# xbpeng/DeepMimic

Hardware: NVIDIA H100
Metric: env-steps/sec (30 Hz policy steps; humanoid3d_spinkick, 4096 envs/GPU) (higher is better)
Workload: dtype f32

## Files before the change

### deepmimic_b200/csrc/kernels/dm_step.cu

```cuda
#include "dm_model.cuh"
#include <type_traits>

namespace dmk {

namespace {

template <int W>
struct Tl {
    static __device__ __forceinline__ float shfl(float v, int src) { return __shfl_sync(0xffffffffu, v, src, W); }
    static __device__ __forceinline__ int shfli(int v, int src) { return __shfl_sync(0xffffffffu, v, src, W); }
    static __device__ __forceinline__ V3 shfl3(V3 v, int src) { return mk3(shfl(v.x, src), shfl(v.y, src), shfl(v.z, src)); }
    static __device__ __forceinline__ S6 shfl6(S6 v, int src) { return mks(shfl3(v.a, src), shfl3(v.l, src)); }
};
__device__ __forceinline__ void ld12(const float* p, float* o) {
    const float4 a = reinterpret_cast<const float4*>(p)[0], b = reinterpret_cast<const float4*>(p)[1], c_ = reinterpret_cast<const float4*>(p)[2];
    o[0] = a.x; o[1] = a.y; o[2] = a.z; o[3] = a.w; o[4] = b.x; o[5] = b.y; o[6] = b.z; o[7] = b.w; o[8] = c_.x; o[9] = c_.y; o[10] = c_.z; o[11] = c_.w;
}
__device__ __forceinline__ void st12(float* p, const float* o) {
    reinterpret_cast<float4*>(p)[0] = make_float4(o[0], o[1], o[2], o[3]); reinterpret_cast<float4*>(p)[1] = make_float4(o[4], o[5], o[6], o[7]);
    reinterpret_cast<float4*>(p)[2] = make_float4(o[8], o[9], o[10], o[11]);
}
__device__ __forceinline__ float rcp_fast(float x) { float r; asm("rcp.approx.ftz.f32 %0, %1;" : "=f"(r) : "f"(x)); return r; }
__device__ __forceinline__ int wmax(int v) {
#pragma unroll
// ... 69 lines not shown
int dm_step_layout(int nl, int n, int chain_len, int maxrows, int W, StepLayout* L) {
    const int maxpts = maxrows / 3;
    int o = 0;
    L->nl = nl; L->n = n; L->chain_len = chain_len; L->maxrows = maxrows; L->maxpts = maxpts;
    L->oU = o; o += nl * 24;
    L->oR = o; o += nl * 12;
    L->oA = o;
    const int world = nl * 24, tri = maxrows * (maxrows + 1) / 2;
    L->oW = o; L->oV = o + nl * 12;
    L->oPp = o + world; L->oQ = L->oPp + maxpts * 4;
    const int pre = world + maxpts * 4 + 4 * 8;
    o += (pre > tri ? pre : tri);
    o = (o + 3) & ~3;
    const int ys = dm_step_y_stride(W), scr = 28 * (nl - 1);
    L->oY = o; o += (chain_len * ys > scr) ? chain_len * ys : scr;
    L->oLam = o; o += maxrows; o += (o & 1); L->oRhs = o; o += maxrows; L->oInv = o; o += maxrows;
    L->oRl = o; o += maxrows;
    L->oPi = o; o += maxpts; L->oPr = o; o += maxpts;
    L->oG = o; o += 21 + 13 + 2;
    L->oZ = o; o += ((n + 3) / 4) * 4;
    L->env_floats = ((o + 15) / 32) * 32 + 16;
    L->hot_floats = kHdrFloats + ((nl * kLkFloats + (nl * nl + nl * chain_len + 3) / 4 + 3) / 4) * 4;
    return L->hot_floats * 4 + 0;
}
int dm_step_smem_bytes(const StepLayout& L, int tiles) { return (L.hot_floats + L.env_floats * tiles) * static_cast<int>(sizeof(float)); }

constexpr int kPgsBlock = 2;
enum PgsSection { kSecLimit = 0, kSecNormal = 1, kSecFriction = 2 };
template <int W, int S, int ST, int B>
__device__ __forceinline__ void pgs_sweeps(const float* sA, float* sLam, const float2* sRI, int lane, int NL, int P, int NLmax, int Pmax, float mu) {
    using T = Tl<W>;
    float w[S];
#pragma unroll
    for (int s = 0; s < S; ++s) w[s] = 0.f;
    int tjs[S];
#pragma unroll
    for (int s = 0; s < S; ++s) { const int rid = lane + s * W; tjs[s] = rid * (rid + 1) / 2; }
    auto tri = [](int i) { return (i * (i + 1)) >> 1; };
    auto a_own = [&](int s, int i, int ti) -> float {
        if (ST > 0) return sA[i * ST + lane + s * W];
        const int rid = lane + s * W;
        return sA[(rid >= i) ? (tjs[s] + i) : (ti + rid)];
    };
    auto a_pair = [&](int i, int j, int ti, int tj_) -> float {
        if (ST > 0) return sA[i * ST + j];
        return sA[(i >= j) ? (ti + j) : (tj_ + i)];
    };
#pragma unroll 1
    for (int p = 0; p < Pmax; ++p) {
        const int i = NL + ((p < P) ? p : 0);
        const float l0 = (p < P) ? sLam[i] : 0.f;
#pragma unroll
        for (int s = 0; s < S; ++s) w[s] = fmaf(a_own(s, i, tri(i)), l0, w[s]);
    }
    bool writer[B];
#pragma unroll
    for (int k = 0; k < B; ++k) writer[k] = lane == k;
    auto block = [&](int pos0, int it, auto sec_tag) {
        constexpr int SEC = decltype(sec_tag)::value;
        int ik[B], tk[B]; bool vk[B];
        float tot = 0.f;
        float wk[B], rhs[B], inv[B], lam[B], lo[B], hi[B], ain[B * (B - 1) / 2 > 0 ? B * (B - 1) / 2 : 1], ao[S][B];
        if (SEC == kSecLimit) {
#pragma unroll
            for (int k = 0; k < B; ++k) { const int pos = pos0 + k; vk[k] = pos < NL; ik[k] = vk[k] ? ((it & 1) ? pos : NL - 1 - pos) : 0; }
        } else {
            const int i0 = ((SEC == kSecNormal) ? NL : NL + P) + pos0, cnt = (SEC == kSecNormal) ? P : 2 * P;
#pragma unroll
            for (int k = 0; k < B; ++k) { ik[k] = i0 + k; vk[k] = pos0 + k < cnt; }
        }
#pragma unroll
        for (int k = 0; k < B; ++k) tk[k] = (ST > 0) ? 0 : tri(ik[k]);
#pragma unroll
        for (int k = 0; k < B; ++k) {
            const float2 ri = sRI[ik[k]];
            rhs[k] = ri.x; inv[k] = ri.y; lam[k] = sLam[ik[k]];
            if (SEC == kSecFriction) {
                if ((B & 1) != 0 || (k & 1) == 0) tot = sLam[NL + ((pos0 + k) >> 1)];
                const bool on = tot > 0.f;
                hi[k] = on ? mu * tot : lam[k]; lo[k] = on ? -hi[k] : lam[k];
            } else { lo[k] = 0.f; hi[k] = (SEC == kSecLimit) ? 100.f : 1e10f; }
        }
        {
            int o = 0;
#pragma unroll
            for (int k = 1; k < B; ++k)
#pragma unroll
                for (int j = 0; j < k; ++j) ain[o++] = a_pair(ik[k], ik[j], tk[k], tk[j]);
        }
#pragma unroll
        for (int s = 0; s < S; ++s)
#pragma unroll
            for (int k = 0; k < B; ++k) ao[s][k] = a_own(s, ik[k], tk[k]);
#pragma unroll
        for (int k = 0; k < B; ++k) {
            float sel = w[0];
#pragma unroll
            for (int s = 1; s < S; ++s) if (ik[k] >= s * W) sel = w[s];
            wk[k] = T::shfl(sel, (S == 1) ? ik[k] : (ik[k] & (W - 1)));
        }
#pragma unroll
        for (int k = 0; k < B; ++k) {
            float c = fmaxf(fmaf(-inv[k], wk[k], rhs[k]), lo[k] - lam[k]);
            if (SEC != kSecNormal) c = fminf(c, hi[k] - lam[k]);
            c = vk[k] ? c : 0.f;
#pragma unroll
            for (int j = k + 1; j < B; ++j) wk[j] = fmaf(ain[j * (j - 1) / 2 + k], c, wk[j]);
            if (vk[k] && writer[k]) sLam[ik[k]] = (SEC == kSecNormal) ? fmaxf(lam[k] + c, 0.f) : fminf(fmaxf(lam[k] + c, lo[k]), hi[k]);
#pragma unroll
            for (int s = 0; s < S; ++s) w[s] = fmaf(ao[s][k], c, w[s]);
        }
        __syncwarp();
    };
#pragma unroll 1
    for (int it = 0; it < 10; ++it) {
#pragma unroll 1
        for (int p0 = 0; p0 < NLmax; p0 += B) block(p0, it, std::integral_constant<int, kSecLimit>{});
#pragma unroll 1
        for (int p0 = 0; p0 < Pmax; p0 += B) block(p0, it, std::integral_constant<int, kSecNormal>{});
#pragma unroll 1
        for (int p0 = 0; p0 < 2 * Pmax; p0 += B) block(p0, it, std::integral_constant<int, kSecFriction>{});
    }
}

template <int W>
__device__ __noinline__ void solve_rows(int NL, int P, float* mani, int alive, unsigned int* prf) {
    using T = Tl<W>;
    float* const sm_ = step_smem();
    const int* LYS = reinterpret_cast<const int*>(sm_ + kHLayout);
    const float* LK = sm_ + kHdrFloats;
    const int lane = threadIdx.x % W;
    const float h = sm_[kHh], mu = sm_[kHMu];
#ifdef DM_PROFILE
    unsigned int pt = static_cast<unsigned int>(clock64());
#define SPROF(sec) do { if ((threadIdx.x & 31) == 0) { unsigned int t_ = static_cast<unsigned int>(clock64()); prf[sec] += t_ - pt; pt = t_; } } while (0)
#else
#define SPROF(sec) do { } while (0)
#endif
    const StepLayout& LY = *reinterpret_cast<const StepLayout*>(LYS);
    const int nl = LY.nl, CL = LY.chain_len, MR = LY.maxrows;
    constexpr int YS = dm_step_y_stride(W);
    float* const E = sm_ + LY.hot_floats + (threadIdx.x / W) * LY.env_floats;
    const unsigned char* CD = reinterpret_cast<const unsigned char*>(LK + nl * kLkFloats);
    const unsigned char* CH = CD + nl * nl;
    float* sU = E + LY.oU; float* sS = E + LY.oR; float* sW = E + LY.oW; float* sV = E + LY.oV; float* sA = E + LY.oA; float* sY = E + LY.oY;
    float* sLam = E + LY.oLam; float2* sRI = reinterpret_cast<float2*>(E + LY.oRhs); int* sRl = reinterpret_cast<int*>(E + LY.oRl);
    float* sPp = E + LY.oPp; float* sPi = E + LY.oPi; int* sPr = reinterpret_cast<int*>(E + LY.oPr);
    float* sQ = E + LY.oQ; float* sG = E + LY.oG; float* sZ = E + LY.oZ;
    auto lk_i = [&](int j) { return reinterpret_cast<const int*>(LK + j * kLkFloats)[kLInt]; };
    auto lk_i2 = [&](int j) { return reinterpret_cast<const int*>(LK + j * kLkFloats)[kLInt2]; };
    auto shift_f = [](S6 f, V3 c) { return mks(f.a + cross(c, f.l), f.l); };
    const int NR = NL + 3 * P;
    const int NRmax = (W == 32) ? NR : wmax(NR);
    const int nslots = (NRmax + W - 1) / W;
    constexpr int kSlots = 2;
#pragma unroll
    for (int s = 0; s < kSlots; ++s) {
        const int rid = lane + s * W;
        if (s < nslots) {
            const bool rv_ = rid < NR;
            int b = 0, kind = 0 , p = 0;
            float lsign = 1.f, lpen = 0.f;
            if (rv_) {
                if (rid < NL) { b = __float_as_int(sQ[rid]); lsign = sQ[8 + rid]; lpen = sQ[16 + rid]; }
                else if (rid < NL + P) { kind = 1; p = rid - NL; b = sPr[p] >> 2; }
                else { const int f = rid - NL - P; p = f >> 1; kind = 2 + (f & 1); b = sPr[p] >> 2; }
                sRl[rid] = b;
            }
            S6 f = mks(mk3(0, 0, 0), mk3(0, 0, 0));
            float rvel = 0.f, pdist = 0.f;
            if (rv_ && kind != 0) {
                const float* w = sW + b * 12;
                pdist = sPp[p * 4 + 3];
                const V3 rel = mk3(sPp[p * 4] - w[9], sPp[p * 4 + 1] - w[10], sPp[p * 4 + 2] - w[11]);
                const V3 fl_ = (kind == 1) ? mk3(0.f, 1.f, 0.f) : ((kind == 2) ? mk3(-1.f, 0.f, 0.f) : mk3(0.f, 0.f, 1.f));
                f = mks(cross(rel, fl_), fl_);
                const float* v = sV + b * 12;
                rvel = dot(fl_, mk3(v[3], v[4], v[5]) + cross(mk3(v[0], v[1], v[2]), rel));
            }
            float acc = 0.f;
            int cur = b;
            bool first = true;
#pragma unroll 1
            while (true) {
                const int info = lk_i(cur);
                const int par = static_cast<int>(static_cast<signed char>(info & 0xff)), nd = (info >> 16) & 0xff, dp0 = (info >> 24) & 0xff;
                const float4* u4 = reinterpret_cast<const float4*>(sU + cur * 24);
                const float4* q4 = reinterpret_cast<const float4*>(sS + cur * 12);
                const float4 ua = u4[0], ub = u4[1], uc = u4[2], ud = u4[3], ue = u4[4], uf = u4[5];
                const float4 qa = q4[0], qb = q4[1], qc = q4[2];
                if (nd == 3) {
                    {
                        const float t = qb.z * f.a.x + qb.w * f.a.y + qc.x * f.a.z;
                        const float y = t * uf.w;
                        if (rv_) sY[(dp0 + 2) * YS + rid] = y;
                        acc += y * y;
                        const float ti = t * uf.x;
                        f.a.x -= ti * ud.x; f.a.y -= ti * ud.y; f.a.z -= ti * ud.z; f.l.x -= ti * ud.w; f.l.y -= ti * ue.x; f.l.z -= ti * ue.y;
                    }
                    {
                        const float t = qa.w * f.a.x + qb.x * f.a.y + qb.y * f.a.z;
                        const float y = t * uf.z;
                        if (rv_) sY[(dp0 + 1) * YS + rid] = y;
                        acc += y * y;
                        const float ti = t * ue.w;
                        f.a.x -= ti * ub.z; f.a.y -= ti * ub.w; f.a.z -= ti * uc.x; f.l.x -= ti * uc.y; f.l.y -= ti * uc.z; f.l.z -= ti * uc.w;
                    }
                }
                if (nd >= 1) {
                    float t = qa.x * f.a.x + qa.y * f.a.y + qa.z * f.a.z;
                    if (first && kind == 0) { t = lsign; rvel = lsign * sQ[24 + rid]; }
                    const float y = t * uf.y;
                    if (rv_) sY[dp0 * YS + rid] = y;
                    acc += y * y;
                    const float ti = t * ue.z;
                    f.a.x -= ti * ua.x; f.a.y -= ti * ua.y; f.a.z -= ti * ua.z; f.l.x -= ti * ua.w; f.l.y -= ti * ub.x; f.l.z -= ti * ub.y;
                }
                first = false;
                f = shift_f(f, mk3(qc.y, qc.z, qc.w));
                if (par < 0) break;
                cur = par;
            }
            {
                float x[6] = {f.a.x, f.a.y, f.a.z, f.l.x, f.l.y, f.l.z};
                int o = 0;
#pragma unroll
                for (int i = 0; i < 6; ++i) {
#pragma unroll
                    for (int k = 0; k < i; ++k) x[i] -= sG[o++] * x[k];
                    x[i] *= sG[15 + i];
                    if (rv_) sY[i * YS + rid] = x[i];
                    acc += x[i] * x[i];
                }
            }
            if (rv_) {
                const float inv = acc > 1.1920929e-7f ? 1.0f / acc : 0.f;
                float rhs, lam0 = 0.f;
                if (kind == 1) {
                    float perr = 0.f, verr = -rvel;
                    if (pdist > 0.f) verr -= pdist / h; else perr = -pdist * 0.2f / h;
                    rhs = perr * inv + verr * inv;
                    lam0 = sPi[p] * 0.85f;
                } else if (kind != 0) rhs = -rvel * inv;
                else {
                    float perr = 0.f, verr = -rvel;
                    const bool combine = lpen > -0.04f;
                    if (lpen > 0.f) verr = -lpen / h; else perr = -lpen * 0.2f / h;
                    rhs = combine ? (perr * inv + verr * inv) : (verr * inv);
                }
                sRI[rid] = make_float2(rhs, inv); sLam[rid] = lam0;
            }
        }
    }
    __syncwarp();
    SPROF(7);
    const int Pmax = (W == 32) ? P : wmax(P);
    const int NLmax = (W == 32) ? NL : wmax(NL);
    {
        constexpr int kSq2 = (W == 16) ? 22 : 36;
        const int region = max(nl * 24, MR * (MR + 1) / 2);
        const int mode = (nslots == 1) ? 0 : ((NRmax <= kSq2 && kSq2 * kSq2 + W <= region) ? 1 : 2);
        const int st = (mode == 0) ? W : kSq2;
        auto put = [&](int i, int j, float v) {
            if (mode != 2) { sA[i * st + j] = v; sA[j * st + i] = v; }
            else { const int hi_ = max(i, j), lo_ = min(i, j); sA[hi_ * (hi_ + 1) / 2 + lo_] = v; }
        };
#pragma unroll 1
        for (int j = 0; j < NLmax; ++j) {
            const bool jv = j < NL;
            const int bj = jv ? sRl[j] : 0;
#pragma unroll 1
            for (int i0 = 0; i0 < NRmax; i0 += W) {
                const int i = i0 + lane;
                const bool pv = jv && i < NR && i >= j;
                const int cd = pv ? CD[sRl[i] * nl + bj] : 0;
                const float* yi = sY + (pv ? i : 0); const float* yj = sY + (jv ? j : 0);
                float acc = 0.f;
#pragma unroll 1
                for (int k = 0; k < CL; k += 4, yi += 4 * YS, yj += 4 * YS) {
                    const float a0 = yi[0], a1 = yi[YS], a2 = yi[2 * YS], a3 = yi[3 * YS];
                    const float b0 = yj[0], b1 = yj[YS], b2 = yj[2 * YS], b3 = yj[3 * YS];
                    if (k < cd) acc += a0 * b0;
                    if (k + 1 < cd) acc += a1 * b1;
                    if (k + 2 < cd) acc += a2 * b2;
                    if (k + 3 < cd) acc += a3 * b3;
                }
                if (pv) put(i, j, acc);
            }
        }
        const int npp = P * (P + 1) / 2, nppmax = Pmax * (Pmax + 1) / 2;
#pragma unroll 1
        for (int q0 = 0; q0 < nppmax; q0 += W) {
            const int q = q0 + lane;
            const bool pv = q < npp;
            int pp = static_cast<int>((sqrtf(8.0f * static_cast<float>(q) + 1.0f) - 1.0f) * 0.5f);
            if (pp * (pp + 1) / 2 > q) --pp;
            if ((pp + 1) * (pp + 2) / 2 <= q) ++pp;
            const int pr = q - pp * (pp + 1) / 2;
            const int in_p = pv ? NL + pp : 0, it_p = pv ? NL + P + 2 * pp : 0, in_r = pv ? NL + pr : 0, it_r = pv ? NL + P + 2 * pr : 0;
            const int cd = pv ? CD[sRl[in_p] * nl + sRl[in_r]] : 0;
            const float* ypn = sY + in_p; const float* ypt = sY + it_p; const float* yrn = sY + in_r; const float* yrt = sY + it_r;
            float acc[3][3];
#pragma unroll
            for (int x = 0; x < 3; ++x)
#pragma unroll
                for (int y = 0; y < 3; ++y) acc[x][y] = 0.f;
#pragma unroll 1
            for (int k = 0; k < CL; k += 4, ypn += 4 * YS, ypt += 4 * YS, yrn += 4 * YS, yrt += 4 * YS) {
                float av[3][4], bv[3][4];
#pragma unroll
                for (int d = 0; d < 4; ++d) {
                    av[0][d] = ypn[d * YS]; av[1][d] = ypt[d * YS]; av[2][d] = ypt[d * YS + 1];
                    bv[0][d] = yrn[d * YS]; bv[1][d] = yrt[d * YS]; bv[2][d] = yrt[d * YS + 1];
                }
#pragma unroll
                for (int d = 0; d < 4; ++d)
                    if (k + d < cd) {
#pragma unroll
                        for (int x = 0; x < 3; ++x)
#pragma unroll
                            for (int y = 0; y < 3; ++y) acc[x][y] += av[x][d] * bv[y][d];
                    }
            }
            if (pv) {
                if (mode != 2) {
                    float* rp[3] = {sA + in_p * st, sA + it_p * st, sA + it_p * st + st};
                    float* rr[3] = {sA + in_r * st, sA + it_r * st, sA + it_r * st + st};
                    const int cp[3] = {in_p, it_p, it_p + 1}, cr[3] = {in_r, it_r, it_r + 1};
#pragma unroll
                    for (int x = 0; x < 3; ++x)
#pragma unroll
                        for (int y = 0; y < 3; ++y) { rp[x][cr[y]] = acc[x][y]; rr[y][cp[x]] = acc[x][y]; }
                } else {
#pragma unroll
                    for (int x = 0; x < 3; ++x)
#pragma unroll
                        for (int y = 0; y < 3; ++y) put(x == 0 ? in_p : it_p + x - 1, y == 0 ? in_r : it_r + y - 1, acc[x][y]);
                }
            }
        }
        __syncwarp();
        SPROF(8);
        if (mode == 0) pgs_sweeps<W, 1, W, kPgsBlock>(sA, sLam, sRI, lane, NL, P, NLmax, Pmax, mu);
        else if (mode == 1) pgs_sweeps<W, kSlots, kSq2, kPgsBlock>(sA, sLam, sRI, lane, NL, P, NLmax, Pmax, mu);
        else pgs_sweeps<W, kSlots, 0, kPgsBlock>(sA, sLam, sRI, lane, NL, P, NLmax, Pmax, mu);
    }
    SPROF(9);
#pragma unroll 1
    for (int p = lane; p < P; p += W) {
        if (alive) {
            const int ref = sPr[p];
            float* mpt = mani + (ref >> 2) * kManifoldFloats + (ref & 3) * 12;
            mpt[7] = sLam[NL + p]; mpt[8] = sLam[NL + P + 2 * p]; mpt[9] = sLam[NL + P + 2 * p + 1];
        }
    }
    {
        const int info = (lane < nl) ? lk_i(lane) : 0;
        const int nd = (info >> 16) & 0xff, dp0 = (info >> 24) & 0xff;
        const int d0 = (lane < nl) ? (lk_i2(lane) & 0xff) : 0;
        float z0 = 0.f, z1 = 0.f, z2 = 0.f, zb = 0.f;
        const int kb = (lane < 6) ? lane : 0;
        const bool mine = lane < nl && nd > 0;
        const int need = dp0 + nd - 1;
        const unsigned char* cdl = CD + lane;
#pragma unroll 2
        for (int i = 0; i < NRmax; ++i) {
            const int b = sRl[i];
            const float l = (i < NR) ? sLam[i] : 0.f;
            const float yb = sY[kb * YS + i], y0 = sY[dp0 * YS + i], y1 = sY[(dp0 + 1) * YS + i], y2 = sY[(dp0 + 2) * YS + i];
            const bool in = mine && cdl[b * nl] > need;
            zb = fmaf(yb, l, zb);
            if (in) { z0 = fmaf(y0, l, z0); if (nd == 3) { z1 = fmaf(y1, l, z1); z2 = fmaf(y2, l, z2); } }
        }
        if (lane < 6) sZ[lane] = zb;
        if (lane < nl && nd >= 1) sZ[d0] = z0;
        if (lane < nl && nd == 3) { sZ[d0 + 1] = z1; sZ[d0 + 2] = z2; }
    }
    __syncwarp();
}


struct Ctx {
    float* E;
    const int* LYS;
    const float* LK;
    int lane, li;
    int plane, level, ndof, jtype, maxlevel;
    bool act;
};
__device__ __forceinline__ const StepLayout& lay_of(const Ctx& c) { return *reinterpret_cast<const StepLayout*>(c.LYS); }
template <int W>
__device__ __forceinline__ Ctx make_ctx() {
    Ctx c;
    float* sm = step_smem();
    c.LYS = reinterpret_cast<const int*>(sm + kHLayout); c.LK = sm + kHdrFloats;
    const StepLayout& LY = *reinterpret_cast<const StepLayout*>(c.LYS);
    const int tile = threadIdx.x / W;
    c.lane = threadIdx.x % W;
    c.act = c.lane < LY.nl;
    c.li = c.act ? c.lane : LY.nl - 1;
    c.E = sm + LY.hot_floats + tile * LY.env_floats;
    const int* q = reinterpret_cast<const int*>(c.LK + c.li * kLkFloats);
    const int info = q[kLInt], tree = q[kLTree];
    const int par = static_cast<int>(static_cast<signed char>(info & 0xff));
    c.plane = par >= 0 ? par : 0; c.jtype = (info >> 8) & 0xff; c.ndof = c.act ? ((info >> 16) & 0xff) : 0;
    c.level = c.act ? (tree & 0xff) : 1000; c.maxlevel = (tree >> 8) & 0xff;
    return c;
}
__device__ __forceinline__ S6 shift_m(S6 m, V3 c) { return mks(m.a, m.l + cross(m.a, c)); }
__device__ __forceinline__ S6 shift_f(S6 f, V3 c) { return mks(f.a + cross(c, f.l), f.l); }
__device__ __forceinline__ float cl100(float v) { return fminf(fmaxf(v, -100.f), 100.f); }
template <int W>
__device__ __forceinline__ V3 tile_com(const float* w, const float* v, float mass, float inv_total) {
    float cx = mass * (w[9] + v[6]), cy = mass * (w[10] + v[7]), cz = mass * (w[11] + v[8]);
#pragma unroll
    for (int o = W / 2; o > 0; o >>= 1) {
        cx += __shfl_xor_sync(0xffffffffu, cx, o, W); cy += __shfl_xor_sync(0xffffffffu, cy, o, W); cz += __shfl_xor_sync(0xffffffffu, cz, o, W);
    }
    return mk3(cx * inv_total, cy * inv_total, cz * inv_total);
}

template <int W>
__device__ __noinline__ void kin_pass(float4 jp, float4 jv) {
    const Ctx c = make_ctx<W>();
    using T = Tl<W>;
    const StepLayout& LY = lay_of(c);
    float* sS = c.E + LY.oR; float* sW = c.E + LY.oW; float* sV = c.E + LY.oV; const float* sB = c.E + LY.oG + 21;
    const float* LKo = c.LK + c.li * kLkFloats;
    const float4 ax4 = ld4(LKo + kLAx), zr4 = ld4(LKo + kLZr), c4 = ld4(LKo + kLC);
    const V3 axis = mk3(ax4.x, ax4.y, ax4.z);
    const Q4 zrot = mkq(zr4.x, zr4.y, zr4.z, zr4.w);
    const V3 cvec = mk3(c4.x, c4.y, c4.z);
    Q4 cached;
    if (c.jtype == kJSpherical) cached = qmul(mkq(jp.x, jp.y, jp.z, -jp.w), zrot);
    else if (c.jtype == kJRevolute) {
        float s, co;
        __sincosf(-0.5f * jp.x, &s, &co);
        cached = qmul(mkq(axis.x * s, axis.y * s, axis.z * s, co), zrot);
    } else cached = zrot;
    const M3 R = qmat(cached);
    V3 jw = mk3(0, 0, 0);
    if (c.jtype == kJSpherical) jw = mk3(jv.x, jv.y, jv.z); else if (c.jtype == kJRevolute) jw = jv.x * axis;
    M3 Rwl; V3 Pw, cw; S6 vel;
    if (c.lane == 0) {
        const M3 Rwb = qmat(mkq(sB[3], sB[4], sB[5], sB[6]));
        const V3 bo = mk3(sB[7], sB[8], sB[9]);
        Rwl = mul(R, Rwb); cw = mulT(Rwb, cvec); Pw = mk3(sB[0], sB[1], sB[2]) + cw;
        vel = mks(bo + mulT(Rwl, jw), mk3(sB[10], sB[11], sB[12]) + cross(bo, cw));
    }
#pragma unroll 1
    for (int lv = 1; lv <= c.maxlevel; ++lv) {
        M3 pR; V3 pp; S6 pv;
#pragma unroll
        for (int k = 0; k < 9; ++k) pR.m[k] = T::shfl(Rwl.m[k], c.plane);
        pp = T::shfl3(Pw, c.plane);
        pv = T::shfl6(vel, c.plane);
        if (c.level == lv) {
            Rwl = mul(R, pR); cw = mulT(pR, cvec); Pw = pp + cw;
            vel = mks(pv.a + mulT(Rwl, jw), pv.l + cross(pv.a, cw));
        }
    }
    if (c.act) {
        const float4 d4 = ld4(LKo + kLD);
        const V3 dw = mulT(Rwl, mk3(d4.x, d4.y, d4.z));
        V3 S0 = mk3(Rwl.m[0], Rwl.m[1], Rwl.m[2]);
        if (c.jtype != kJSpherical) S0 = mulT(Rwl, axis);
        const float wr[12] = {Rwl.m[0], Rwl.m[1], Rwl.m[2], Rwl.m[3], Rwl.m[4], Rwl.m[5], Rwl.m[6], Rwl.m[7], Rwl.m[8], Pw.x, Pw.y, Pw.z};
        const float qr[12] = {S0.x, S0.y, S0.z, Rwl.m[3], Rwl.m[4], Rwl.m[5], Rwl.m[6], Rwl.m[7], Rwl.m[8], cw.x, cw.y, cw.z};
        const float vr[12] = {vel.a.x, vel.a.y, vel.a.z, vel.l.x, vel.l.y, vel.l.z, dw.x, dw.y, dw.z, 0.f, 0.f, 0.f};
        st12(sW + c.lane * 12, wr); st12(sS + c.lane * 12, qr); st12(sV + c.lane * 12, vr);
    }
    __syncwarp();
}

template <int W>
__device__ __noinline__ int collide(float* mani, int alive, int mcnt) {
    const Ctx c = make_ctx<W>();
    const float scale = step_smem()[kHScale];
    using T = Tl<W>;
    const StepLayout& LY = lay_of(c);
    const float* sW = c.E + LY.oW; const float* sV = c.E + LY.oV;
    float* sPp = c.E + LY.oPp; float* sPi = c.E + LY.oPi; int* sPr = reinterpret_cast<int*>(c.E + LY.oPr);
    const float* LKo = c.LK + c.li * kLkFloats;
    const int shape = reinterpret_cast<const int*>(LKo)[kLFlg] & 0xff;
    int cnt = 0;
    float mp[48];
    M3 Rwl;
    float wrec[12], vrec[12];
    ld12(sW + c.li * 12, wrec); ld12(sV + c.li * 12, vrec);
#pragma unroll
    for (int k = 0; k < 9; ++k) Rwl.m[k] = wrec[k];
    const float thr = LKo[kLThr];
    const float4 he4 = ld4(LKo + kLHe);
    const V3 he = mk3(he4.x, he4.y, he4.z);
    const V3 pos = mk3(wrec[9] + vrec[6], wrec[10] + vrec[7], wrec[11] + vrec[8]);
    V3 dl = mul(Rwl, mk3(0.f, -1.f, 0.f));
    V3 vtx;
    if (shape == kSBox) vtx = mk3(dl.x >= 0 ? he.x : -he.x, dl.y >= 0 ? he.y : -he.y, dl.z >= 0 ? he.z : -he.z);
    else {
        V3 sup = mk3(0, 0, 0);
        if (shape == kSCapsule) sup = mk3(0.f, (dl.y >= 0.f) ? he.y : -he.y, 0.f);
        float inv = rsqrtf(dot(dl, dl));
        vtx = sup + (he.x * inv) * dl;
    }
    const V3 vw = pos + mulT(Rwl, vtx);
    const float dist = vw.y;
    const bool need = c.act && alive && (mcnt > 0 || dist < thr);
    {
        const float4* mg = reinterpret_cast<const float4*>(mani + c.li * kManifoldFloats);
#pragma unroll
        for (int k = 0; k < 12; ++k) { float4 v = need ? mg[k] : make_float4(0.f, 0.f, 0.f, 0.f); mp[4 * k] = v.x; mp[4 * k + 1] = v.y; mp[4 * k + 2] = v.z; mp[4 * k + 3] = v.w; }
    }
#pragma unroll
    for (int k = 0; k < 4; ++k) if (mp[k * 12] != 0.f && cnt == k) cnt = k + 1;
    if (c.act && dist < thr) {
        float best = thr * thr; int nearest = -1;
#pragma unroll
        for (int k = 0; k < 4; ++k) if (k < cnt) {
// ... 562 lines not shown
                    if (kind == kTaskStrike) {
                        const double scene_time = tm[kTTimer];
                        tk[kKTimer] += dt;
                        strike_update(M.taskx, tk, tkx, rx, rz, scene_time, B);
                        if (tk[kKTimer] >= tk[kKTimerMax]) task_timer_reset(M.task, tk, rng);
                        tf = strike_terminate(M.task, M.taskx, tk, tkx, rx, rz, scene_time);
                    } else {
                        task_update(task_base_kind(kind), M.task, tk, rng, dt, rx, rz);
                        tf = task_dist_fail(kind, M.task, tk, rx, rz) ? 1 : 0;
                        if (kind == kTaskHeadingGetup) {
                            tkx[kXHeadY] = B.head_y;
                            if (getup_update(M.taskx, tkx, dt, M.test_mode != 0, fallen != 0)) fe = 0;
                        }
                    }
                }
                task_fail = T::shfli(tf, 0);
                fallen_eff = T::shfli(fe, 0);
            }
            if (alive) {
                int term = (M.enable_fall_end && fallen_eff) ? 1 : 0;
                if (!term && (cbits & 4)) term = 1;
                if (TASK && !term && task_fail) term = task_fail;
                f_updates++;
                const bool end = (cbits & 2) || term;
                if (end || stage == total_stages) {
                    if (lane == 0) {
                        reinterpret_cast<float4*>(sim)[0] = make_float4(sB[0], sB[1], sB[2], 0.f);
                        reinterpret_cast<float4*>(sim)[1] = make_float4(sB[3], sB[4], sB[5], sB[6]);
                        reinterpret_cast<float4*>(sim)[2] = make_float4(sB[7], sB[8], sB[9], 0.f);
                        reinterpret_cast<float4*>(sim)[3] = make_float4(sB[10], sB[11], sB[12], 0.f);
                        fl[kFNeedAction] = need_action; fl[kFDone] = end ? 1 : 0; fl[kFTerminate] = term; fl[kFValid] = (eseg == 0) ? 1 : 0; fl[kFFallen] = fallen_eff;
                        fl[kFRowOverflow] = f_over; fl[kFUpdates] = f_updates;
                    }
                    if (act) {
                        reinterpret_cast<float4*>(sim + 16)[lane] = jp;
                        reinterpret_cast<float4*>(sim + 16 + 4 * nl)[lane] = jv;
                    }
                }
                if (end) alive = false;
            }
        }
        PROF(1);
        if (stage == total_stages) break;
        if (__syncthreads_and(!alive)) break;
        PROF(2);
        if (__ballot_sync(0xffffffffu, alive) == 0u) continue;
        const int ph = stage % stages_per_upd;
        if (ph == 0) {
            int cb = 0;
            if constexpr (TASK) {
                if (__ballot_sync(0xffffffffu, alive && need_action) != 0u) {
                    const V3 com = tile_com<W>(E + LY.oW + li * 12, sV + li * 12, act ? LKo[kLM] : 0.f, 1.0f / (M.total_mass * scale));
                    if (lane == 0 && alive && need_action) { tk[kKPrevCom] = com.x; tk[kKPrevCom + 1] = com.y; tk[kKPrevCom + 2] = com.z; }
                }
            }
            if (lane == 0 && alive) {
                const double timer = tm[kTTimer] + dt;
                double kin_time = tm[kTKin];
                double dur_ = M.motion_dur;
                if constexpr (TASK) dur_ = st.ctab->info[st.clip[env]].dur;
                const double dur = dur_;
                double p0 = kin_time / dur; p0 -= floor(p0);
                kin_time += dt;
                double p1 = kin_time / dur; p1 -= floor(p1);
                if constexpr (TASK) {
                    const ClipInfo& ci = st.ctab->info[st.clip[env]];
                    if (ci.loop && p1 < p0 && M.sync_root_pos) {
                        const double simq[4] = {static_cast<double>(sB[3]), static_cast<double>(sB[4]), static_cast<double>(sB[5]), static_cast<double>(sB[6])};
                        kin_wrap_sync(frame_times + ci.frame_off, frames + static_cast<size_t>(ci.frame_off) * M.pose_dim, M.pose_dim, ci.num_frames, ci.cycle_delta, dur, kin_time,
                                      tm + kTOrigin, tm + kTOriginRot, static_cast<double>(sB[0]) / M.scale, static_cast<double>(sB[2]) / M.scale, simq, true, false);
                    }
                } else if (M.loop_motion && p1 < p0 && (M.sync_root_pos || M.sync_root_rot)) {
                    const double simq[4] = {static_cast<double>(sB[3]), static_cast<double>(sB[4]), static_cast<double>(sB[5]), static_cast<double>(sB[6])};
                    kin_wrap_sync(frame_times, frames, M.pose_dim, M.num_frames, M.cycle_delta, dur, kin_time, tm + kTOrigin, tm + kTOriginRot,
                                  static_cast<double>(sB[0]) / M.scale, static_cast<double>(sB[2]) / M.scale, simq, M.sync_root_pos != 0, M.sync_root_rot != 0);
                }
                const double ctrl_time = tm[kTCtrl] + dt;
                if (need_action) tm[kTPrevAct] = ctrl_time;
                tm[kTTimer] = timer; tm[kTKin] = kin_time; tm[kTCtrl] = ctrl_time;
                {
                    const double cur = ctrl_time + tm[kTInitOff], pad = 0.001 * dt, T_ = M.query_dt;
                    int c0 = static_cast<int>(floor((cur + pad) / T_)), c1 = static_cast<int>(floor((cur + pad - dt) / T_));
                    cb = (c0 != c1) ? 1 : 0;
                }
                if (timer >= tm[kTTimerMax]) cb |= 2;
                if (M.end_at_clip_end && kin_time >= dur) cb |= 4;
            }
            cbits = T::shfli(cb, 0);
            need_action = 0;
            PROF(3);
            const float4 tg = reinterpret_cast<const float4*>(sim + 16 + 8 * nl)[li];
            float e0 = 0, e1 = 0, e2 = 0;
            if (jtype == kJSpherical) {
                Q4 q = mkq(jp.x, jp.y, jp.z, jp.w);
                Q4 dq = qmul(q, mkq(jv.x, jv.y, jv.z, 0.f));
                Q4 qi = qnormalize(mkq(q.x + 0.5f * fdt * dq.x, q.y + 0.5f * fdt * dq.y, q.z + 0.5f * fdt * dq.z, q.w + 0.5f * fdt * dq.w));
                V3 e = quat_rotvec3(qmul(qconj(qi), mkq(tg.x, tg.y, tg.z, tg.w)));
                e0 = e.x; e1 = e.y; e2 = e.z;
            } else if (jtype == kJRevolute) {
                e0 = tg.x - (normalize_angle3(jp.x) + fdt * jv.x);
            }
            const float kp = LKo[kLKp], kd = LKo[kLKd];
            const float pe0 = kp * e0, pe1 = kp * e1, pe2 = kp * e2;
            const float3 qdd = aba_solve<W>(pe0 - kd * jv.x, pe1 - kd * jv.y, pe2 - kd * jv.z, fdt * kd, 0, jv.x, jv.y, jv.z);
            float t0 = 0, t1 = 0, t2 = 0;
            if (ndof >= 1) t0 = pe0 + kd * (-jv.x - fdt * qdd.x);
            if (ndof == 3) { t1 = pe1 + kd * (-jv.y - fdt * qdd.y); t2 = pe2 + kd * (-jv.z - fdt * qdd.z); }
            const float mag = sqrtf(t0 * t0 + t1 * t1 + t2 * t2), tlim = LKo[kLTl];
            if (mag > tlim) { float s = tlim / mag; t0 *= s; t1 *= s; t2 *= s; }
            tau0 = t0; tau1 = t1; tau2 = t2;
            PROF(4);
            continue;
        }
        int P;
        {
            const int r = collide<W>(mani, alive ? 1 : 0, mcnt);
            P = r & 0xff; in_contact_tol = ((r >> 8) & 1) != 0; if ((r >> 9) & 1) f_over = 1; mcnt = (r >> 10) & 7;
        }
        PROF(3);
        {
            const float3 qdd = aba_solve<W>(tau0, tau1, tau2, 0.f, 1, jv.x, jv.y, jv.z);
            bool hit = false;
            if (ndof >= 1) { const float v = jv.x + h * qdd.x; jv.x = cl100(v); hit |= fabsf(v) > 100.f; }
            if (ndof == 3) { const float v1 = jv.y + h * qdd.y, v2 = jv.z + h * qdd.z; jv.y = cl100(v1); jv.z = cl100(v2); hit |= fabsf(v1) > 100.f || fabsf(v2) > 100.f; }
            if (lane == 0) for (int k = 0; k < 6; ++k) hit |= fabsf(sB[7 + k]) >= 100.f;
            const unsigned hb = __ballot_sync(0xffffffffu, hit);
            if (hb != 0u) {
                const unsigned hseg = (W == 32) ? hb : ((hb >> (threadIdx.x & 16)) & 0xffffu);
                vel_pass<W>(jv.x, jv.y, jv.z, hseg != 0u);
            }
        }
        PROF(4);
        int lim_dir = 0; float lim_pen = 0.f;
        if (act && has_limit && alive) {
            float p0 = jp.x - LKo[kLLo], p1 = LKo[kLHi] - jp.x;
            if (!(p0 > 0.f)) { lim_dir = 1; lim_pen = p0; }
            else if (!(p1 > 0.f)) { lim_dir = -1; lim_pen = p1; }
        }
        const unsigned lbal = __ballot_sync(0xffffffffu, lim_dir != 0);
        const unsigned lseg = (W == 32) ? lbal : ((lbal >> (threadIdx.x & 16)) & 0xffffu);
        int NL = __popc(lseg);
        const unsigned anyrow = __ballot_sync(0xffffffffu, NL + P > 0);
        if (anyrow != 0) {
            {
                const int lidx = __popc(lseg & ((1u << lane) - 1u));
                if (NL > 8) { NL = 8; f_over = 1; }
                if (lim_dir != 0 && lidx < 8) { sQ[lidx] = __int_as_float(lane); sQ[8 + lidx] = (lim_dir == -1) ? -1.f : 1.f; sQ[16 + lidx] = lim_pen; sQ[24 + lidx] = jv.x; }
            }
            if (NL + 3 * P > LY.maxrows) { P = (LY.maxrows - NL) / 3; f_over = 1; }
            const int NR = NL + 3 * P;
            __syncwarp();
            PROF(5);
#ifdef DM_PROFILE
            { const int nrm = wmax(NR); if ((threadIdx.x & 31) == 0) { PRF[13] += nrm; PRF[14] += 1; if (nrm > W) PRF[15] += 1; } }
#endif
            solve_rows<W>(NL, P, mani, alive ? 1 : 0, PRFP);
            PROF(10);
            const float3 dq = dv_pass<W>();
            if (NR > 0) {
                if (ndof >= 1) jv.x = cl100(jv.x + dq.x);
                if (ndof == 3) { jv.y = cl100(jv.y + dq.y); jv.z = cl100(jv.z + dq.z); }
            }
            PROF(11);
        }
        if (lane == 0) {
            sB[0] += h * sB[10]; sB[1] += h * sB[11]; sB[2] += h * sB[12];
            const Q4 q = quat_integrate3(mk3(sB[7], sB[8], sB[9]), mkq(sB[3], sB[4], sB[5], sB[6]), true, h);
            sB[3] = q.x; sB[4] = q.y; sB[5] = q.z; sB[6] = q.w;
        }
        if (jtype == kJRevolute) jp.x += h * jv.x;
        else if (jtype == kJSpherical) { Q4 q = quat_integrate3(mk3(jv.x, jv.y, jv.z), mkq(jp.x, jp.y, jp.z, jp.w), false, h); jp = make_float4(q.x, q.y, q.z, q.w); }
        __syncwarp();
        need_kin = true;
        if (ph == sim_substeps) pending_flags = true;
        PROF(12);
    }
#ifdef DM_PROFILE
    __syncwarp();
    if ((threadIdx.x & 31) == 0 && st.prof) { unsigned int* o = st.prof + (blockIdx.x * (blockDim.x / 32) + threadIdx.x / 32) * kProfCounters; for (int k = 0; k < kProfCounters; ++k) o[k] = PRF[k]; }
#endif
}

template __global__ void dm_step_kernel<16, false>(const DevModel*, DevState, const double*, const float*, double, int, int, StepLayout);
template __global__ void dm_step_kernel<32, false>(const DevModel*, DevState, const double*, const float*, double, int, int, StepLayout);
template __global__ void dm_step_kernel<16, true>(const DevModel*, DevState, const double*, const float*, double, int, int, StepLayout);
template __global__ void dm_step_kernel<32, true>(const DevModel*, DevState, const double*, const float*, double, int, int, StepLayout);

}
```

Before: 2.342 million.

## Solve each half-warp env serially with full warp when rows exceed half-warp

In the W=16 half-warp-per-env path, when one env has more constraint rows than 16 but both fit in 32, the warp now processes the two envs one after another using all 32 lanes. This avoids the two-slot row layout and packed/square-matrix PGS modes with half-warp granularity, using a single-slot 32-wide PGS instead. Row building and A assembly are refactored into lambdas parameterized on the env base pointer. It also raises the unroll of the impulse accumulation loop for W=16; the trade-off is serializing two envs, which can cost time when both envs have many rows.

Result: faster. 2.409 million, median of 6 (+2.8%).

```diff
diff --git a/deepmimic_b200/csrc/kernels/dm_step.cu b/deepmimic_b200/csrc/kernels/dm_step.cu
--- a/deepmimic_b200/csrc/kernels/dm_step.cu
+++ b/deepmimic_b200/csrc/kernels/dm_step.cu
@@ -245,129 +245,124 @@
     auto shift_f = [](S6 f, V3 c) { return mks(f.a + cross(c, f.l), f.l); };
     const int NR = NL + 3 * P;
     const int NRmax = (W == 32) ? NR : wmax(NR);
-    const int nslots = (NRmax + W - 1) / W;
-    constexpr int kSlots = 2;
-#pragma unroll
-    for (int s = 0; s < kSlots; ++s) {
-        const int rid = lane + s * W;
-        if (s < nslots) {
-            const bool rv_ = rid < NR;
-            int b = 0, kind = 0 , p = 0;
-            float lsign = 1.f, lpen = 0.f;
-            if (rv_) {
-                if (rid < NL) { b = __float_as_int(sQ[rid]); lsign = sQ[8 + rid]; lpen = sQ[16 + rid]; }
-                else if (rid < NL + P) { kind = 1; p = rid - NL; b = sPr[p] >> 2; }
-                else { const int f = rid - NL - P; p = f >> 1; kind = 2 + (f & 1); b = sPr[p] >> 2; }
-                sRl[rid] = b;
-            }
-            S6 f = mks(mk3(0, 0, 0), mk3(0, 0, 0));
-            float rvel = 0.f, pdist = 0.f;
-            if (rv_ && kind != 0) {
-                const float* w = sW + b * 12;
-                pdist = sPp[p * 4 + 3];
-                const V3 rel = mk3(sPp[p * 4] - w[9], sPp[p * 4 + 1] - w[10], sPp[p * 4 + 2] - w[11]);
-                const V3 fl_ = (kind == 1) ? mk3(0.f, 1.f, 0.f) : ((kind == 2) ? mk3(-1.f, 0.f, 0.f) : mk3(0.f, 0.f, 1.f));
-                f = mks(cross(rel, fl_), fl_);
-                const float* v = sV + b * 12;
-                rvel = dot(fl_, mk3(v[3], v[4], v[5]) + cross(mk3(v[0], v[1], v[2]), rel));
-            }
-            float acc = 0.f;
-            int cur = b;
-            bool first = true;
-#pragma unroll 1
-            while (true) {
-                const int info = lk_i(cur);
-                const int par = static_cast<int>(static_cast<signed char>(info & 0xff)), nd = (info >> 16) & 0xff, dp0 = (info >> 24) & 0xff;
-                const float4* u4 = reinterpret_cast<const float4*>(sU + cur * 24);
-                const float4* q4 = reinterpret_cast<const float4*>(sS + cur * 12);
-                const float4 ua = u4[0], ub = u4[1], uc = u4[2], ud = u4[3], ue = u4[4], uf = u4[5];
-                const float4 qa = q4[0], qb = q4[1], qc = q4[2];
-                if (nd == 3) {
-                    {
-                        const float t = qb.z * f.a.x + qb.w * f.a.y + qc.x * f.a.z;
-                        const float y = t * uf.w;
-                        if (rv_) sY[(dp0 + 2) * YS + rid] = y;
-                        acc += y * y;
-                        const float ti = t * uf.x;
-                        f.a.x -= ti * ud.x; f.a.y -= ti * ud.y; f.a.z -= ti * ud.z; f.l.x -= ti * ud.w; f.l.y -= ti * ue.x; f.l.z -= ti * ue.y;
-                    }
-                    {
-                        const float t = qa.w * f.a.x + qb.x * f.a.y + qb.y * f.a.z;
-                        const float y = t * uf.z;
-                        if (rv_) sY[(dp0 + 1) * YS + rid] = y;
-                        acc += y * y;
-                        const float ti = t * ue.w;
-                        f.a.x -= ti * ub.z; f.a.y -= ti * ub.w; f.a.z -= ti * uc.x; f.l.x -= ti * uc.y; f.l.y -= ti * uc.z; f.l.z -= ti * uc.w;
-                    }
+    auto in_blk = [&](float* Eb, int off, float* own) -> float* { if constexpr (W == 16) return Eb + off; else return own; };
+    auto build_row = [&](float* Eb, int rid, bool rv_, int NL, int P) {
+        const float* sUe = in_blk(Eb, LY.oU, sU); const float* sSe = in_blk(Eb, LY.oR, sS); const float* sWe = in_blk(Eb, LY.oW, sW);
+        const float* sVe = in_blk(Eb, LY.oV, sV); const float* sPpe = in_blk(Eb, LY.oPp, sPp); const float* sPie = in_blk(Eb, LY.oPi, sPi);
+        const int* sPre = reinterpret_cast<const int*>(in_blk(Eb, LY.oPr, reinterpret_cast<float*>(sPr))); const float* sQe = in_blk(Eb, LY.oQ, sQ);
+        const float* sGe = in_blk(Eb, LY.oG, sG); float* sYe = in_blk(Eb, LY.oY, sY); float* sLame = in_blk(Eb, LY.oLam, sLam);
+        float2* sRIe = reinterpret_cast<float2*>(in_blk(Eb, LY.oRhs, reinterpret_cast<float*>(sRI))); int* sRle = reinterpret_cast<int*>(in_blk(Eb, LY.oRl, reinterpret_cast<float*>(sRl)));
+        int b = 0, kind = 0 , p = 0;
+        float lsign = 1.f, lpen = 0.f;
+        if (rv_) {
+            if (rid < NL) { b = __float_as_int(sQe[rid]); lsign = sQe[8 + rid]; lpen = sQe[16 + rid]; }
+            else if (rid < NL + P) { kind = 1; p = rid - NL; b = sPre[p] >> 2; }
+            else { const int f = rid - NL - P; p = f >> 1; kind = 2 + (f & 1); b = sPre[p] >> 2; }
+            sRle[rid] = b;
+        }
+        S6 f = mks(mk3(0, 0, 0), mk3(0, 0, 0));
+        float rvel = 0.f, pdist = 0.f;
+        if (rv_ && kind != 0) {
+            const float* w = sWe + b * 12;
+            pdist = sPpe[p * 4 + 3];
+            const V3 rel = mk3(sPpe[p * 4] - w[9], sPpe[p * 4 + 1] - w[10], sPpe[p * 4 + 2] - w[11]);
+            const V3 fl_ = (kind == 1) ? mk3(0.f, 1.f, 0.f) : ((kind == 2) ? mk3(-1.f, 0.f, 0.f) : mk3(0.f, 0.f, 1.f));
+            f = mks(cross(rel, fl_), fl_);
+            const float* v = sVe + b * 12;
+            rvel = dot(fl_, mk3(v[3], v[4], v[5]) + cross(mk3(v[0], v[1], v[2]), rel));
+        }
+        float acc = 0.f;
+        int cur = b;
+        bool first = true;
+#pragma unroll 1
+        while (true) {
+            const int info = lk_i(cur);
+            const int par = static_cast<int>(static_cast<signed char>(info & 0xff)), nd = (info >> 16) & 0xff, dp0 = (info >> 24) & 0xff;
+            const float4* u4 = reinterpret_cast<const float4*>(sUe + cur * 24);
+            const float4* q4 = reinterpret_cast<const float4*>(sSe + cur * 12);
+            const float4 ua = u4[0], ub = u4[1], uc = u4[2], ud = u4[3], ue = u4[4], uf = u4[5];
+            const float4 qa = q4[0], qb = q4[1], qc = q4[2];
+            if (nd == 3) {
+                {
+                    const float t = qb.z * f.a.x + qb.w * f.a.y + qc.x * f.a.z;
+                    const float y = t * uf.w;
+                    if (rv_) sYe[(dp0 + 2) * YS + rid] = y;
+                    acc += y * y;
+                    const float ti = t * uf.x;
+                    f.a.x -= ti * ud.x; f.a.y -= ti * ud.y; f.a.z -= ti * ud.z; f.l.x -= ti * ud.w; f.l.y -= ti * ue.x; f.l.z -= ti * ue.y;
                 }
-                if (nd >= 1) {
-                    float t = qa.x * f.a.x + qa.y * f.a.y + qa.z * f.a.z;
-                    if (first && kind == 0) { t = lsign; rvel = lsign * sQ[24 + rid]; }
-                    const float y = t * uf.y;
-                    if (rv_) sY[dp0 * YS + rid] = y;
+                {
+                    const float t = qa.w * f.a.x + qb.x * f.a.y + qb.y * f.a.z;
+                    const float y = t * uf.z;
+                    if (rv_) sYe[(dp0 + 1) * YS + rid] = y;
                     acc += y * y;
-                    const float ti = t * ue.z;
-                    f.a.x -= ti * ua.x; f.a.y -= ti * ua.y; f.a.z -= ti * ua.z; f.l.x -= ti * ua.w; f.l.y -= ti * ub.x; f.l.z -= ti * ub.y;
+                    const float ti = t * ue.w;
+                    f.a.x -= ti * ub.z; f.a.y -= ti * ub.w; f.a.z -= ti * uc.x; f.l.x -= ti * uc.y; f.l.y -= ti * uc.z; f.l.z -= ti * uc.w;
                 }
-                first = false;
-                f = shift_f(f, mk3(qc.y, qc.z, qc.w));
-                if (par < 0) break;
-                cur = par;
-            }
-            {
-                float x[6] = {f.a.x, f.a.y, f.a.z, f.l.x, f.l.y, f.l.z};
-                int o = 0;
-#pragma unroll
-                for (int i = 0; i < 6; ++i) {
-#pragma unroll
-                    for (int k = 0; k < i; ++k) x[i] -= sG[o++] * x[k];
-                    x[i] *= sG[15 + i];
-                    if (rv_) sY[i * YS + rid] = x[i];
-                    acc += x[i] * x[i];
-                }
-            }
-            if (rv_) {
-                const float inv = acc > 1.1920929e-7f ? 1.0f / acc : 0.f;
-                float rhs, lam0 = 0.f;
-                if (kind == 1) {
-                    float perr = 0.f, verr = -rvel;
-                    if (pdist > 0.f) verr -= pdist / h; else perr = -pdist * 0.2f / h;
-                    rhs = perr * inv + verr * inv;
-                    lam0 = sPi[p] * 0.85f;
-                } else if (kind != 0) rhs = -rvel * inv;
-                else {
-                    float perr = 0.f, verr = -rvel;
-                    const bool combine = lpen > -0.04f;
-                    if (lpen > 0.f) verr = -lpen / h; else perr = -lpen * 0.2f / h;
-                    rhs = combine ? (perr * inv + verr * inv) : (verr * inv);
-                }
-                sRI[rid] = make_float2(rhs, inv); sLam[rid] = lam0;
-            }
-        }
-    }
-    __syncwarp();
-    SPROF(7);
-    const int Pmax = (W == 32) ? P : wmax(P);
-    const int NLmax = (W == 32) ? NL : wmax(NL);
-    {
-        constexpr int kSq2 = (W == 16) ? 22 : 36;
-        const int region = max(nl * 24, MR * (MR + 1) / 2);
-        const int mode = (nslots == 1) ? 0 : ((NRmax <= kSq2 && kSq2 * kSq2 + W <= region) ? 1 : 2);
+            }
+            if (nd >= 1) {
+                float t = qa.x * f.a.x + qa.y * f.a.y + qa.z * f.a.z;
+                if (first && kind == 0) { t = lsign; rvel = lsign * sQe[24 + rid]; }
+                const float y = t * uf.y;
+                if (rv_) sYe[dp0 * YS + rid] = y;
+                acc += y * y;
+                const float ti = t * ue.z;
+                f.a.x -= ti * ua.x; f.a.y -= ti * ua.y; f.a.z -= ti * ua.z; f.l.x -= ti * ua.w; f.l.y -= ti * ub.x; f.l.z -= ti * ub.y;
+            }
+            first = false;
+            f = shift_f(f, mk3(qc.y, qc.z, qc.w));
+            if (par < 0) break;
+            cur = par;
+        }
+        {
+            float x[6] = {f.a.x, f.a.y, f.a.z, f.l.x, f.l.y, f.l.z};
+            int o = 0;
+#pragma unroll
+            for (int i = 0; i < 6; ++i) {
+#pragma unroll
+                for (int k = 0; k < i; ++k) x[i] -= sGe[o++] * x[k];
+                x[i] *= sGe[15 + i];
+                if (rv_) sYe[i * YS + rid] = x[i];
+                acc += x[i] * x[i];
+            }
+        }
+        if (rv_) {
+            const float inv = acc > 1.1920929e-7f ? 1.0f / acc : 0.f;
+            float rhs, lam0 = 0.f;
+            if (kind == 1) {
+                float perr = 0.f, verr = -rvel;
+                if (pdist > 0.f) verr -= pdist / h; else perr = -pdist * 0.2f / h;
+                rhs = perr * inv + verr * inv;
+                lam0 = sPie[p] * 0.85f;
+            } else if (kind != 0) rhs = -rvel * inv;
+            else {
+                float perr = 0.f, verr = -rvel;
+                const bool combine = lpen > -0.04f;
+                if (lpen > 0.f) verr = -lpen / h; else perr = -lpen * 0.2f / h;
+                rhs = combine ? (perr * inv + verr * inv) : (verr * inv);
+            }
+            sRIe[rid] = make_float2(rhs, inv); sLame[rid] = lam0;
+        }
+    };
+    constexpr int kSq2 = (W == 16) ? 22 : 36;
+    const int region = max(nl * 24, MR * (MR + 1) / 2);
+    auto build_A = [&](float* Eb, int ln, int nlanes, int NL, int P, int NR, int NLmax, int Pmax, int NRmax, int mode) {
+        float* sAe = in_blk(Eb, LY.oA, sA); const float* sYe = in_blk(Eb, LY.oY, sY); const int* sRle = reinterpret_cast<const int*>(in_blk(Eb, LY.oRl, reinterpret_cast<float*>(sRl)));
         const int st = (mode == 0) ? W : kSq2;
         auto put = [&](int i, int j, float v) {
-            if (mode != 2) { sA[i * st + j] = v; sA[j * st + i] = v; }
-            else { const int hi_ = max(i, j), lo_ = min(i, j); sA[hi_ * (hi_ + 1) / 2 + lo_] = v; }
+            if (mode != 2) { sAe[i * st + j] = v; sAe[j * st + i] = v; }
+            else { const int hi_ = max(i, j), lo_ = min(i, j); sAe[hi_ * (hi_ + 1) / 2 + lo_] = v; }
         };
 #pragma unroll 1
         for (int j = 0; j < NLmax; ++j) {
             const bool jv = j < NL;
-            const int bj = jv ? sRl[j] : 0;
-#pragma unroll 1
-            for (int i0 = 0; i0 < NRmax; i0 += W) {
-                const int i = i0 + lane;
+            const int bj = jv ? sRle[j] : 0;
+#pragma unroll 1
+            for (int i0 = 0; i0 < NRmax; i0 += nlanes) {
+                const int i = i0 + ln;
                 const bool pv = jv && i < NR && i >= j;
-                const int cd = pv ? CD[sRl[i] * nl + bj] : 0;
-                const float* yi = sY + (pv ? i : 0); const float* yj = sY + (jv ? j : 0);
+                const int cd = pv ? CD[sRle[i] * nl + bj] : 0;
+                const float* yi = sYe + (pv ? i : 0); const float* yj = sYe + (jv ? j : 0);
                 float acc = 0.f;
 #pragma unroll 1
                 for (int k = 0; k < CL; k += 4, yi += 4 * YS, yj += 4 * YS) {
@@ -383,16 +378,16 @@
         }
         const int npp = P * (P + 1) / 2, nppmax = Pmax * (Pmax + 1) / 2;
 #pragma unroll 1
-        for (int q0 = 0; q0 < nppmax; q0 += W) {
-            const int q = q0 + lane;
+        for (int q0 = 0; q0 < nppmax; q0 += nlanes) {
+            const int q = q0 + ln;
             const bool pv = q < npp;
             int pp = static_cast<int>((sqrtf(8.0f * static_cast<float>(q) + 1.0f) - 1.0f) * 0.5f);
             if (pp * (pp + 1) / 2 > q) --pp;
             if ((pp + 1) * (pp + 2) / 2 <= q) ++pp;
             const int pr = q - pp * (pp + 1) / 2;
             const int in_p = pv ? NL + pp : 0, it_p = pv ? NL + P + 2 * pp : 0, in_r = pv ? NL + pr : 0, it_r = pv ? NL + P + 2 * pr : 0;
-            const int cd = pv ? CD[sRl[in_p] * nl + sRl[in_r]] : 0;
-            const float* ypn = sY + in_p; const float* ypt = sY + it_p; const float* yrn = sY + in_r; const float* yrt = sY + it_r;
+            const int cd = pv ? CD[sRle[in_p] * nl + sRle[in_r]] : 0;
+            const float* ypn = sYe + in_p; const float* ypt = sYe + it_p; const float* yrn = sYe + in_r; const float* yrt = sYe + it_r;
             float acc[3][3];
 #pragma unroll
             for (int x = 0; x < 3; ++x)
@@ -417,8 +412,8 @@
             }
             if (pv) {
                 if (mode != 2) {
-                    float* rp[3] = {sA + in_p * st, sA + it_p * st, sA + it_p * st + st};
-                    float* rr[3] = {sA + in_r * st, sA + it_r * st, sA + it_r * st + st};
+                    float* rp[3] = {sAe + in_p * st, sAe + it_p * st, sAe + it_p * st + st};
+                    float* rr[3] = {sAe + in_r * st, sAe + it_r * st, sAe + it_r * st + st};
                     const int cp[3] = {in_p, it_p, it_p + 1}, cr[3] = {in_r, it_r, it_r + 1};
 #pragma unroll
                     for (int x = 0; x < 3; ++x)
@@ -433,12 +428,53 @@
             }
         }
         __syncwarp();
+    };
+    bool serial = false;
+    if constexpr (W == 16) serial = NRmax > W && -wmax(-NR) <= W;
+    if (serial) {
+        if constexpr (W == 16) {
+            const int lw = threadIdx.x & 31;
+#pragma unroll 1
+            for (int e = 0; e < 2; ++e) {
+                const int NLe = __shfl_sync(0xffffffffu, NL, 16 * e), Pe = __shfl_sync(0xffffffffu, P, 16 * e), NRe = NLe + 3 * Pe;
+                if (NRe == 0) continue;
+                float* const Ee = sm_ + LY.hot_floats + ((threadIdx.x >> 5) * 2 + e) * LY.env_floats;
+                build_row(Ee, lw, lw < NRe, NLe, Pe);
+                __syncwarp();
+                SPROF(7);
+                const int mode = (NRe <= kSq2 && kSq2 * kSq2 + 32 <= region) ? 1 : 2;
+                build_A(Ee, lw, 32, NLe, Pe, NRe, NLe, Pe, NRe, mode);
+                SPROF(8);
+                const float2* RIe = reinterpret_cast<const float2*>(Ee + LY.oRhs);
+                if (mode == 1) pgs_sweeps<32, 1, kSq2, kPgsBlock>(Ee + LY.oA, Ee + LY.oLam, RIe, lw, NLe, Pe, NLe, Pe, mu);
+                else pgs_sweeps<32, 1, 0, kPgsBlock>(Ee + LY.oA, Ee + LY.oLam, RIe, lw, NLe, Pe, NLe, Pe, mu);
+                SPROF(9);
+            }
+        }
+    } else {
+        const int nslots = (NRmax + W - 1) / W;
+        constexpr int kSlots = 2;
+#pragma unroll
+        for (int s = 0; s < kSlots; ++s) {
+            const int rid = lane + s * W;
+            if (s < nslots) build_row(E, rid, rid < NR, NL, P);
+        }
+        __syncwarp();
+        SPROF(7);
+        const int Pmax = (W == 32) ? P : wmax(P);
+        const int NLmax = (W == 32) ? NL : wmax(NL);
+        const int mode = (nslots == 1) ? 0 : ((NRmax <= kSq2 && kSq2 * kSq2 + W <= region) ? 1 : 2);
+        build_A(E, lane, W, NL, P, NR, NLmax, Pmax, NRmax, mode);
         SPROF(8);
         if (mode == 0) pgs_sweeps<W, 1, W, kPgsBlock>(sA, sLam, sRI, lane, NL, P, NLmax, Pmax, mu);
         else if (mode == 1) pgs_sweeps<W, kSlots, kSq2, kPgsBlock>(sA, sLam, sRI, lane, NL, P, NLmax, Pmax, mu);
         else pgs_sweeps<W, kSlots, 0, kPgsBlock>(sA, sLam, sRI, lane, NL, P, NLmax, Pmax, mu);
     }
     SPROF(9);
+    if constexpr (W == 16) {
+        float* const Ez = sm_ + LY.hot_floats + (threadIdx.x / W) * LY.env_floats;
+        sY = Ez + LY.oY; sLam = Ez + LY.oLam; sRl = reinterpret_cast<int*>(Ez + LY.oRl); sPr = reinterpret_cast<int*>(Ez + LY.oPr); sZ = Ez + LY.oZ;
+    }
 #pragma unroll 1
     for (int p = lane; p < P; p += W) {
         if (alive) {
@@ -456,7 +492,7 @@
         const bool mine = lane < nl && nd > 0;
         const int need = dp0 + nd - 1;
         const unsigned char* cdl = CD + lane;
-#pragma unroll 2
+#pragma unroll (W == 16 ? 4 : 2)
         for (int i = 0; i < NRmax; ++i) {
             const int b = sRl[i];
             const float l = (i < NR) ? sLam[i] : 0.f;
@@ -1325,7 +1361,10 @@
             __syncwarp();
             PROF(5);
 #ifdef DM_PROFILE
-            { const int nrm = wmax(NR); if ((threadIdx.x & 31) == 0) { PRF[13] += nrm; PRF[14] += 1; if (nrm > W) PRF[15] += 1; } }
+            {
+                const int nrm = wmax(NR), nenv = __popc(__ballot_sync(0xffffffffu, NR > 0)) / W;
+                if ((threadIdx.x & 31) == 0) { PRF[13] += nrm; PRF[14] += 1; if (nrm > W) PRF[15] += nenv; }
+            }
 #endif
             solve_rows<W>(NL, P, mani, alive ? 1 : 0, PRFP);
             PROF(10);
```
